# dr-tony-lin/CarND-MPC-Project

Hardware: AMD Instinct MI355X
Metric: MPC solves/sec (batch) at N=10 dt=0.1 (higher is better)
Workload: dtype f64

## Files before the change

### carnd-mpc-project_amd/csrc/mpc_core.h

```cpp
#ifndef MPC_CORE_H
#define MPC_CORE_H

#include <math.h>
#include <stdint.h>
#include <type_traits>

#include "mpc_amd.h"

#if defined(__HIPCC__)
#define MPC_HD __host__ __device__ __forceinline__
#else
#define MPC_HD inline
#endif
#if defined(__HIPCC__) || defined(__clang__)
#define MPC_UNROLL _Pragma("unroll")
#define MPC_STAGE_LOOP _Pragma("clang loop unroll(disable)")
#else
#define MPC_UNROLL _Pragma("GCC unroll 8")
#define MPC_STAGE_LOOP
#endif

namespace mpc {

template <class R> struct Layout;
// ... 13 lines not shown
    SOC_C = 0, SOC_D = 6, SOC_SZ = SOC_D + D_N
  };
  static_assert((int)GAIN_SZ <= (int)L::IT_SZ, "the gains must fit an iterate slot");
  static_assert(L::F_ZL % L::G == 0 && L::F_ZU == L::F_ZL + 4 && L::F_U == L::F_S + 6, "blocks the forward sweep fetches");
};

MPC_HD int64_t workspace_fields_per_instance(int N, bool f32, bool s0_rows = false) {
  return (int64_t)(N - 1 + (s0_rows ? 1 : 0)) * (f32 ? (int)Fields<float>::STAGE_SZ : (int)Fields<double>::STAGE_SZ);
}
MPC_HD int64_t soc_fields_per_instance(int N) { return (int64_t)(N - 1) * (int)Fields<double>::SOC_SZ; }

template <class R>
struct HostWorkspace {
  using F = Fields<R>;
  static constexpr bool kSocDefault = true;
  R *base;
  mutable R socbuf[(MPC_MAX_N - 1) * F::SOC_SZ] = {};
  MPC_HD R &soc(int k, int f) const { return socbuf[k * F::SOC_SZ + f]; }
  MPC_HD R &it(int k, int I, int f) const { return base[k * F::STAGE_SZ + I + f]; }
  MPC_HD R getD(int k, int j) const { return base[k * F::STAGE_SZ + F::F_D + j]; }
  MPC_HD void setD(int k, int j, R v) const { base[k * F::STAGE_SZ + F::F_D + j] = v; }
  template <int F0, int COUNT> MPC_HD void store_run(int k, int I, const R *v) const {
    for (int j = 0; j < COUNT; j++) base[k * F::STAGE_SZ + I + F0 + j] = v[j];
  }
  MPC_HD void stage_fetch_it(int, int, int) const {}
  MPC_HD void stage_fetch_itf(int, int, int) const {}
  MPC_HD void stage_fetch_d(int, int) const {}
  template <int N> MPC_HD void stage_wait() const {}
  MPC_HD void stage_drain() const {}
  MPC_HD R sit(int, int k, int I, int j) const { return base[k * F::STAGE_SZ + I + j]; }
  MPC_HD R sx(int, int k, int Fo, int j) const { return base[k * F::STAGE_SZ + Fo + j]; }
  MPC_HD void stage_fetch_g(int, int, int) const {}
  MPC_HD R sg(int, int k, int J, int j) const { return base[k * F::STAGE_SZ + J + F::F_GK + j]; }
};

#if defined(__HIPCC__)
#if defined(__HIP_DEVICE_COMPILE__)
typedef __attribute__((address_space(1))) double gdouble;
typedef __attribute__((address_space(1))) float gfloat;
typedef __attribute__((address_space(1))) char gchar;
typedef __attribute__((address_space(3))) double ldouble;
typedef __attribute__((address_space(3))) float lfloat;
typedef __attribute__((address_space(3))) char lchar;
#else
typedef double gdouble;
typedef float gfloat;
typedef char gchar;
typedef double ldouble;
typedef float lfloat;
typedef char lchar;
#endif
#if defined(__HIP_DEVICE_COMPILE__)
__device__ __forceinline__ unsigned mpc_uniform(unsigned x) {
  unsigned s = (unsigned)__builtin_amdgcn_readfirstlane((int)x);
  asm volatile("" : "+s"(s));
  return s;
}
#define MPC_UNIFORM(x) mpc_uniform((unsigned)(x))
#else
#define MPC_UNIFORM(x) ((unsigned)(x))
#endif
template <class R> struct AddrSpace;
template <> struct AddrSpace<double> { typedef gdouble g; typedef ldouble l; };
template <> struct AddrSpace<float> { typedef gfloat g; typedef lfloat l; };

template <bool STAGING, class R, bool LANE_ROWS = false>
struct TiledWorkspace {
  static_assert(!(STAGING && LANE_ROWS), "LDS-DMA copies record k of every lane from a scalar base: per-lane rows are not staged");
  using F = Fields<R>;
  typedef typename AddrSpace<R>::g greal;
  typedef typename AddrSpace<R>::l lreal;
  static constexpr bool kSocDefault = false;
  greal *tile;
  lreal *lbuf;
  int lane;
  static constexpr unsigned G = F::G;
  static constexpr unsigned GROUPS = F::STAGE_SZ / F::G;
  static_assert(F::STAGE_SZ % F::G == 0 && F::IT_SZ % F::G == 0, "whole groups");
  MPC_HD gchar *row(int k, int f) const {
    if constexpr (LANE_ROWS) return (gchar *)tile + (((unsigned)k * GROUPS + ((unsigned)f / G)) * 1024u + ((unsigned)f % G) * (unsigned)sizeof(R));
    else return (gchar *)tile + MPC_UNIFORM(((unsigned)k * GROUPS + ((unsigned)f / G)) * 1024u + ((unsigned)f % G) * (unsigned)sizeof(R));
  }
  MPC_HD unsigned voff(int I) const { return (unsigned)lane * 16u + ((unsigned)I / G) * 1024u; }
  MPC_HD greal &it(int k, int I, int f) const { return *(greal *)(row(k, f) + voff(I)); }
  template <int F0, int COUNT> MPC_HD void store_run(int k, int I, const R *v) const {
    static_assert(F0 % F::G == 0 && COUNT % F::G == 0, "whole groups");
    typedef R __attribute__((ext_vector_type(16 / sizeof(R)))) vec;
    typedef __attribute__((address_space(1))) vec gvec;
    MPC_UNROLL
    for (int g = 0; g < COUNT / (int)G; g++) {
      vec x;
      MPC_UNROLL
      for (int e = 0; e < (int)G; e++) x[e] = v[g * (int)G + e];
      *(gvec *)(row(k, F0 + g * (int)G) + voff(I)) = x;
    }
  }
  MPC_HD R getD(int k, int j) const { return it(k, 0, F::F_D + j); }
  MPC_HD void setD(int k, int j, R v) const { it(k, 0, F::F_D + j) = v; }
#if defined(MPC_DMA_NT) && MPC_DMA_NT
// ... 18 lines not shown
        asm volatile("s_mov_b32 m0, %2\n\tglobal_load_lds_dwordx4 %0, %1" MPC_DMA_POLICY "\n\tglobal_load_lds_dwordx4 %0, %1 offset:1024" MPC_DMA_POLICY "\n\t"
                     "global_load_lds_dwordx4 %0, %1 offset:2048" MPC_DMA_POLICY
                     :: "v"(vo), "s"(src), "s"(m0v) : "memory", "m0");
      else if (q0 + 2 == n)
        asm volatile("s_mov_b32 m0, %2\n\tglobal_load_lds_dwordx4 %0, %1" MPC_DMA_POLICY "\n\tglobal_load_lds_dwordx4 %0, %1 offset:1024" MPC_DMA_POLICY
                     :: "v"(vo), "s"(src), "s"(m0v) : "memory", "m0");
      else
        asm volatile("s_mov_b32 m0, %2\n\tglobal_load_lds_dwordx4 %0, %1" MPC_DMA_POLICY :: "v"(vo), "s"(src), "s"(m0v) : "memory", "m0");
    }
#endif
  }
  MPC_HD void stage_fetch_it(int buf, int k, int I) const { if (STAGING) dma<F::STG_IT_OPS>(buf, k, I, 0, 0); }
  MPC_HD void stage_fetch_itf(int buf, int k, int I) const {
    if (STAGING) { dma<8 / F::G>(buf, k, I, F::F_S, F::F_S / F::G); dma<8 / F::G>(buf, k, I, F::F_ZL, F::F_ZL / F::G); }
  }
  MPC_HD void stage_fetch_d(int buf, int k) const { if (STAGING) dma<F::STG_D_OPS>(buf, k, 0, F::F_D, F::STG_IT_OPS); }
  MPC_HD void stage_fetch_g(int buf, int k, int J) const { if (STAGING) dma<F::STG_X_OPS>(buf, k, J, F::F_GK, F::STG_IT_OPS); }
  MPC_HD void stage_drain() const {
#if !defined(MPC_NO_DRAIN)
    stage_wait<0>();
#endif
  }
  template <int N> MPC_HD void stage_wait() const {
#if defined(__HIP_DEVICE_COMPILE__)
    if (STAGING) asm volatile("s_waitcnt vmcnt(%0)" ::"n"(N) : "memory");
#endif
  }
  MPC_HD R sl(int buf, int j) const {
    return lbuf[(((unsigned)buf * F::STG_SLOT + ((unsigned)j / G)) * 64u + (unsigned)lane) * G + ((unsigned)j % G)];
  }
  MPC_HD R sit(int buf, int k, int I, int j) const { return STAGING ? sl(buf, j) : (R)it(k, I, j); }
  MPC_HD R sx(int buf, int k, int Fo, int j) const { return STAGING ? sl(buf, F::IT_SZ + j) : (R)it(k, 0, Fo + j); }
  MPC_HD R sg(int buf, int k, int J, int j) const { return STAGING ? sl(buf, F::IT_SZ + j) : (R)it(k, J, F::F_GK + j); }
};
template <bool STAGING, class R>
struct TiledSocWorkspace : TiledWorkspace<STAGING, R> {
  using F = Fields<R>;
  typedef typename AddrSpace<R>::g greal;
  static constexpr bool kSocDefault = true;
  greal *soc_tile;
  MPC_HD greal &soc(int k, int f) const {
    constexpr unsigned G = F::G;
    static_assert(F::SOC_SZ % F::G == 0, "whole groups");
    return soc_tile[(((unsigned)k * (F::SOC_SZ / G) + (unsigned)f / G) * 64u + (unsigned)this->lane) * G + (unsigned)f % G];
  }
};

template <class R, int LANES>
struct LdsWorkspace {
  using F = Fields<R>;
  typedef typename AddrSpace<R>::l lreal;
  static constexpr bool kSocDefault = false;
  lreal *base;
  int lane;
  MPC_HD lreal &it(int k, int I, int f) const { return base[(unsigned)((k * F::STAGE_SZ + I + f) * LANES + lane)]; }
  MPC_HD R getD(int k, int j) const { return it(k, 0, F::F_D + j); }
  MPC_HD void setD(int k, int j, R v) const { it(k, 0, F::F_D + j) = v; }
  template <int F0, int COUNT> MPC_HD void store_run(int k, int I, const R *v) const {
    MPC_UNROLL
    for (int j = 0; j < COUNT; j++) it(k, I, F0 + j) = v[j];
  }
  MPC_HD void stage_fetch_it(int, int, int) const {}
  MPC_HD void stage_fetch_itf(int, int, int) const {}
  MPC_HD void stage_fetch_d(int, int) const {}
  MPC_HD void stage_fetch_g(int, int, int) const {}
  template <int N> MPC_HD void stage_wait() const {}
  MPC_HD void stage_drain() const {}
  MPC_HD R sit(int, int k, int I, int j) const { return it(k, I, j); }
  MPC_HD R sx(int, int k, int Fo, int j) const { return it(k, 0, Fo + j); }
  MPC_HD R sg(int, int k, int J, int j) const { return it(k, J, F::F_GK + j); }
};
template <class R, int LANES>
struct LdsSocWorkspace : LdsWorkspace<R, LANES> {
  using F = Fields<R>;
  typedef typename AddrSpace<R>::l lreal;
  static constexpr bool kSocDefault = true;
  lreal *soc_base;
  MPC_HD lreal &soc(int k, int f) const { return soc_base[(unsigned)((k * F::SOC_SZ + f) * LANES + this->lane)]; }
};
#endif

MPC_HD double frcp(double x) {
#if defined(__HIP_DEVICE_COMPILE__)
  double r = __builtin_amdgcn_rcp(x);
  double e = fma(-x, r, 1.0);
  r = fma(r, e, r);
  e = fma(-x, r, 1.0);
  r = fma(r, e, r);
  return r;
#else
  return 1.0 / x;
#endif
}
#if defined(__HIP_DEVICE_COMPILE__)
template <int LPI> __device__ __forceinline__ int wave_bcast_i(int x, int lane, int base) {
  if constexpr (LPI >= 64) return __builtin_amdgcn_readlane(x, lane);
  else return __builtin_amdgcn_ds_bpermute((base + lane) << 2, x);
}
template <int LPI> __device__ __forceinline__ double wave_bcast(double x, int lane, int base) {
  const int lo = wave_bcast_i<LPI>(__double2loint(x), lane, base), hi = wave_bcast_i<LPI>(__double2hiint(x), lane, base);
  return __hiloint2double(hi, lo);
}
template <int LPI> __device__ __forceinline__ float wave_bcast(float x, int lane, int base) { return __int_as_float(wave_bcast_i<LPI>(__float_as_int(x), lane, base)); }
// ... 626 lines not shown
    R sn[6];
    MPC_UNROLL
    for (int i = 0; i < 6; i++) sn[i] = ws.sit(0, M - 1, I, F_S + i);
    {
      R Hpp, Hvv, Hee, Hcc, gp, gv, ge, gc;
      state_terms(sn[2], sn[3], sn[4], sn[5], ws.sit(0, M - 1, I, F_ZL + 0), ws.sit(0, M - 1, I, F_ZU + 0),
                  ws.sit(0, M - 1, I, F_ZL + 1), ws.sit(0, M - 1, I, F_ZU + 1), Hpp, Hvv, Hee, Hcc, gp, gv, ge, gc);
      Pm[0][0] = hxy; Pm[1][1] = hxy; Pm[2][2] = Hpp + dw; Pm[3][3] = Hvv + dw; Pm[4][4] = Hee + dw;
      Pcc = Hcc + dw; p[2] = gp; p[3] = gv; p[4] = ge; pc = gc;
    }
    R delta = ws.sit(0, M - 1, I, F_U + 0), acc = ws.sit(0, M - 1, I, F_U + 1);
    R lx = ws.sit(0, M - 1, I, F_LAM + 0), ly = ws.sit(0, M - 1, I, F_LAM + 1), lp = ws.sit(0, M - 1, I, F_LAM + 2);
    R lc = ws.sit(0, M - 1, I, F_LAM + 4), le = ws.sit(0, M - 1, I, F_LAM + 5);
    R zld = ws.sit(0, M - 1, I, F_ZL + 2), zud = ws.sit(0, M - 1, I, F_ZU + 2);
    R zla = ws.sit(0, M - 1, I, F_ZL + 3), zua = ws.sit(0, M - 1, I, F_ZU + 3);
    if (M >= 2) ws.stage_fetch_it(1, M - 2, I);
    MPC_STAGE_LOOP
    for (int k = M - 1; k >= 0; --k) {
      R sk[6];
      R zlp = 0, zup = 0, zlv = 0, zuv = 0, delprev = 0;
      const int bk = (M - k) & 1;
      if (k > 0) {
        if (k >= 2) {
          ws.stage_fetch_it(bk ^ 1, k - 2, I);
          if (k == M - 1) ws.template stage_wait<STG_IT_OPS>();
          else ws.template stage_wait<STG_IT_OPS + ST_BACKWARD>();
        } else ws.template stage_wait<0>();
        MPC_UNROLL
        for (int i = 0; i < 6; i++) sk[i] = ws.sit(bk, k - 1, I, F_S + i);
        zlp = ws.sit(bk, k - 1, I, F_ZL + 0); zup = ws.sit(bk, k - 1, I, F_ZU + 0);
        zlv = ws.sit(bk, k - 1, I, F_ZL + 1); zuv = ws.sit(bk, k - 1, I, F_ZU + 1);
        delprev = ws.sit(bk, k - 1, I, F_U + 0);
      } else {
        MPC_UNROLL
        for (int i = 0; i < 6; i++) sk[i] = st[i];
        sk[2] = p0; sk[3] = v0k;
      }
      const R v = sk[3];
      LinR L;
      linearise(sk, delta, acc, sn, L);
      soc_residual(soc, k, L);
      const R sp = L.sp, cp = L.cp, se = L.se, ce = L.ce, fp = L.fp, g1 = L.g1, h3 = L.h3, fpp = L.fpp;
      const R r0 = rsc * L.c[0], r1 = rsc * L.c[1], r2 = rsc * L.c[2], r3 = rsc * L.c[3], rc = rsc * L.c[4], r4 = rsc * L.c[5];
      const R vdt = v * dt;
      const R Axp = -vdt * sp, Axv = dt * cp, Ayp = vdt * cp, Ayv = dt * sp, Apv = delta * dtLf;
      const R Acx = fp, Acv = dt * se, Ace = vdt * ce, Aex = -g1, Bp = v * dtLf;
      R t[6];
      MPC_UNROLL
      for (int i = 0; i < 6; i++)
        t[i] = p[i] + PM(i, 0) * r0 + PM(i, 1) * r1 + PM(i, 2) * r2 + PM(i, 3) * r3 + PM(i, 4) * r4;
      const R tc = pc + Pcc * rc;
      R qt[7];
      MPC_GT(t, tc, qt);
      const R isld = frcp1(delta - dl), isud = frcp1(du - delta), isla = frcp1(acc - al), isua = frcp1(au - acc);
      R ddl = 0, Hdd = 0;
      if (k >= 1 && !lsm) { ddl = delta - delprev; Hdd = df * R(2.0) * wdd; }
      const R mub = lsm ? R(0.0) : mu;
      const R gdel = df * R(2.0) * wd * delta + Hdd * ddl + mub * (isud - isld);
      const R gacc = mub * (isua - isla);
      const R rt_d = qt[5] + gdel, rt_a = qt[6] + gacc;
      const R Sgd = lsm ? R(1.0) : df * R(2.0) * wd + zld * isld + zud * isud, Sga = lsm ? R(1.0) : zla * isla + zua * isua;
      R w5[6], w6[6];
      MPC_UNROLL
      for (int i = 0; i < 6; i++) { w5[i] = Bp * (PM(i, 2) + PM(i, 4)) + PM(i, 5); w6[i] = dt * PM(i, 3); }
      if (k == 0) {
        R o5[7], o6[7];
        MPC_GT(w5, R(0.0), o5);
        MPC_GT(w6, R(0.0), o6);
        const R Rdd = o5[5] + Sgd + dw;
        const R Rda = o6[5];
        const R Raa = o6[6] + Sga + dw;
        const R det = Rdd * Raa - Rda * Rda;
        if (!(Rdd > R(0.0)) || !(det > R(0.0))) return false;
        const R idet = frcp1(det);
        const R i11 = Raa * idet, i12 = -Rda * idet, i22 = Rdd * idet;
        const R Sd2 = o5[2], Sd3 = o5[3] - (lp + le) * dtLf, Sa2 = o6[2], Sa3 = o6[3];
        R gn[GAIN_SZ] = {};
        gn[2] = -(i11 * Sd2 + i12 * Sa2); gn[3] = -(i11 * Sd3 + i12 * Sa3);
        gn[6 + 2] = -(i12 * Sd2 + i22 * Sa2); gn[6 + 3] = -(i12 * Sd3 + i22 * Sa3);
        gn[GK_N] = -(Raa * rt_d - Rda * rt_a) * idet; gn[GK_N + 1] = -(-Rda * rt_d + Rdd * rt_a) * idet;
        ws.template store_run<F_GK, GAIN_SZ>(0, J, gn);
        break;
      }
      R Mx[7][7];
      {
        R w[6], o[7];
        MPC_UNROLL
        for (int i = 0; i < 6; i++) w[i] = PM(i, 0) + Aex * PM(i, 4);
        MPC_GT(w, Pcc * Acx, o);
        MPC_UNROLL
        for (int i = 0; i < 7; i++) Mx[i][0] = o[i];
        MPC_UNROLL
        for (int i = 0; i < 6; i++) w[i] = PM(i, 1);
        MPC_GT(w, -Pcc, o);
        MPC_UNROLL
        for (int i = 0; i < 7; i++) Mx[i][1] = o[i];
        MPC_UNROLL
        for (int i = 0; i < 6; i++) w[i] = Axp * PM(i, 0) + Ayp * PM(i, 1) + PM(i, 2) + PM(i, 4);
        MPC_GT(w, R(0.0), o);
        MPC_UNROLL
        for (int i = 0; i < 7; i++) Mx[i][2] = o[i];
        MPC_UNROLL
        for (int i = 0; i < 6; i++) w[i] = Axv * PM(i, 0) + Ayv * PM(i, 1) + Apv * (PM(i, 2) + PM(i, 4)) + PM(i, 3);
        MPC_GT(w, Pcc * Acv, o);
        MPC_UNROLL
        for (int i = 0; i < 7; i++) Mx[i][3] = o[i];
        {
          const R wcs = Pcc * Ace;
          Mx[0][4] = Acx * wcs; Mx[1][4] = -wcs; Mx[2][4] = R(0.0); Mx[3][4] = Acv * wcs; Mx[4][4] = Ace * wcs;
          Mx[5][4] = R(0.0); Mx[6][4] = R(0.0);
        }
        MPC_GT(w5, R(0.0), o);
        MPC_UNROLL
        for (int i = 0; i < 7; i++) Mx[i][5] = o[i];
// ... 134 lines not shown
    if (s0_rows && !lsm) {
      const R xs0[2] = {p0, v0k}, lo0[2] = {yl, vl}, hi0[2] = {yu, vu}, dx0[2] = {s0d2, s0d3};
      MPC_UNROLL
      for (int b = 0; b < 2; b++) {
        const R isl0 = frcp1(xs0[b] - lo0[b]), isu0 = frcp1(hi0[b] - xs0[b]);
        const R zl0 = s0_z(I, b, 0), zu0 = s0_z(I, b, 1);
        const R dzl = mu * isl0 - zl0 - zl0 * isl0 * dx0[b];
        const R dzu = mu * isu0 - zu0 + zu0 * isu0 * dx0[b];
        rzmax = mpc_max(rzmax, mpc_max(-dzl * frcp1(zl0), -dzu * frcp1(zu0)));
      }
    }
    amax = (rmax > tau) ? tau / rmax : R(1.0);
    az = (rzmax > tau) ? tau / rzmax : R(1.0);
  }

  MPC_HD void forward(bool soc = false) {
    if constexpr (WAVE) { forward_wave(soc); return; }
    const int I = it(cur), J = it(1 - cur);
    R d0 = 0, d1 = 0, d2 = 0, d3 = 0, d5 = 0;
    R ddprev = 0, delprev = 0;
    R rmax = R(0.0), rzmax = R(0.0);
    const R rsc = lsm ? R(0.0) : R(1.0);
    dphi = R(0.0); dxinf = R(0.0); xinf = R(0.0);
    R sk[6];
    load_state(0, I, sk);
    d2 = rsc * (st[2] - p0); d3 = rsc * (st[3] - v0k);
    if (d2 != R(0.0) || d3 != R(0.0)) {
      const R islp = frcp1(p0 - yl), isup = frcp1(yu - p0), islv = frcp1(v0k - vl), isuv = frcp1(vu - v0k);
      rmax = mpc_max(mpc_max(-d2 * islp, d2 * isup), mpc_max(-d3 * islv, d3 * isuv));
      dphi = mu * ((isup - islp) * d2 + (isuv - islv) * d3);
      dxinf = mpc_max(mpc_abs(d2), mpc_abs(d3));
    }
    const R s0d2 = d2, s0d3 = d3;
    ws.stage_drain();
    ws.stage_fetch_itf(0, 0, I);
    ws.stage_fetch_g(0, 0, J);
    R z0lp = R(1.0), z0up = R(1.0), z0lv = R(1.0), z0uv = R(1.0);
    if (s0_rows) { z0lp = s0_z(I, 0, 0); z0up = s0_z(I, 0, 1); z0lv = s0_z(I, 1, 0); z0uv = s0_z(I, 1, 1); }
    MPC_STAGE_LOOP
    for (int k = 0; k < M; ++k) {
      const int bf = k & 1;
      if (k + 1 < M) {
        ws.stage_fetch_itf(bf ^ 1, k + 1, I);
        ws.stage_fetch_g(bf ^ 1, k + 1, J);
        if (k == 0) ws.template stage_wait<STG_ITF_OPS + STG_X_OPS>();
        else ws.template stage_wait<STG_ITF_OPS + STG_X_OPS + ST_FORWARD>();
      } else ws.template stage_wait<0>();
      R sn[6];
      MPC_UNROLL
      for (int i = 0; i < 6; i++) sn[i] = ws.sit(bf, k, I, F_S + i);
      const R v = sk[3];
      const R delta = ws.sit(bf, k, I, F_U + 0), acc = ws.sit(bf, k, I, F_U + 1);
      LinR L;
      linearise(sk, delta, acc, sn, L);
      soc_residual(soc, k, L);
      R dd = ws.sg(bf, k, J, GK_N + 0), da = ws.sg(bf, k, J, GK_N + 1);
      dd += ws.sg(bf, k, J, 0) * d0 + ws.sg(bf, k, J, 1) * d1 + ws.sg(bf, k, J, 2) * d2 + ws.sg(bf, k, J, 3) * d3 +
            ws.sg(bf, k, J, 4) * d5 + ws.sg(bf, k, J, 5) * ddprev;
      da += ws.sg(bf, k, J, 6) * d0 + ws.sg(bf, k, J, 7) * d1 + ws.sg(bf, k, J, 8) * d2 + ws.sg(bf, k, J, 9) * d3 +
            ws.sg(bf, k, J, 10) * d5 + ws.sg(bf, k, J, 11) * ddprev;
      const R vdt = v * dt, Apv = delta * dtLf, Bp = v * dtLf;
      const R n0 = d0 - vdt * L.sp * d2 + dt * L.cp * d3 - rsc * L.c[0];
      const R n1 = d1 + vdt * L.cp * d2 + dt * L.sp * d3 - rsc * L.c[1];
      const R n2 = d2 + Apv * d3 + Bp * dd - rsc * L.c[2];
      const R n3 = d3 + dt * da - rsc * L.c[3];
      const R n4 = L.fp * d0 - d1 + dt * L.se * d3 + vdt * L.ce * d5 - rsc * L.c[4];
      const R n5 = -L.g1 * d0 + d2 + Apv * d3 + Bp * dd - rsc * L.c[5];
      {
        const R dn[D_N] = {n0, n1, n2, n3, n4, n5, dd, da};
        ws.template store_run<F_D, D_N>(k, 0, dn);
      }
      const R q2 = n2, q3 = n3, q4 = n4, q5 = n5, qd = dd, qa = da;
      const R xs[4] = {sn[2], sn[3], delta, acc};
      const R lo[4] = {yl, vl, dl, al}, hi[4] = {yu, vu, du, au};
      const R dx[4] = {q2, q3, qd, qa};
      MPC_UNROLL
      for (int b = 0; b < 4; b++) {
        const R isl = frcp1(xs[b] - lo[b]), isu = frcp1(hi[b] - xs[b]);
        const R zl = ws.sit(bf, k, I, F_ZL + b), zu = ws.sit(bf, k, I, F_ZU + b);
        rmax = mpc_max(rmax, mpc_max(-dx[b] * isl, dx[b] * isu));
        const R dzl = mu * isl - zl - zl * isl * dx[b];
        const R dzu = mu * isu - zu + zu * isu * dx[b];
        rzmax = mpc_max(rzmax, mpc_max(-dzl * frcp1(zl), -dzu * frcp1(zu)));
        dphi += mu * (isu - isl) * dx[b];
      }
      R g = R(2.0) * wc * sn[4] * q4 + R(2.0) * we * sn[5] * q5 + R(2.0) * wv * (sn[3] - vref) * q3 + R(2.0) * wd * delta * qd;
      if (k > 0) g += R(2.0) * wdd * (delta - delprev) * (qd - ddprev);
      dphi += df * g;
      dxinf = mpc_max(dxinf, mpc_max(mpc_max(mpc_max(mpc_abs(n0), mpc_abs(n1)), mpc_max(mpc_abs(n2), mpc_abs(n3))),
                               mpc_max(mpc_max(mpc_abs(n4), mpc_abs(n5)), mpc_max(mpc_abs(dd), mpc_abs(da)))));
      xinf = mpc_max(xinf, mpc_max(mpc_max(mpc_abs(sn[0]), mpc_abs(sn[1])), mpc_max(mpc_abs(sn[3]), mpc_abs(sn[4]))));
      d0 = n0; d1 = n1; d2 = n2; d3 = n3; d5 = n5; ddprev = dd; delprev = delta;
      MPC_UNROLL
      for (int i = 0; i < 6; i++) sk[i] = sn[i];
    }
    if (s0_rows && !lsm) {
      const R xs0[2] = {p0, v0k}, lo0[2] = {yl, vl}, hi0[2] = {yu, vu}, dx0[2] = {s0d2, s0d3};
      const R zl0[2] = {z0lp, z0lv}, zu0[2] = {z0up, z0uv};
      MPC_UNROLL
      for (int b = 0; b < 2; b++) {
        const R isl = frcp1(xs0[b] - lo0[b]), isu = frcp1(hi0[b] - xs0[b]);
        const R dzl = mu * isl - zl0[b] - zl0[b] * isl * dx0[b];
        const R dzu = mu * isu - zu0[b] + zu0[b] * isu * dx0[b];
        rzmax = mpc_max(rzmax, mpc_max(-dzl * frcp1(zl0[b]), -dzu * frcp1(zu0[b])));
      }
    }
    amax = (rmax > tau) ? tau / rmax : R(1.0);
    az = (rzmax > tau) ? tau / rzmax : R(1.0);
  }

  MPC_HD EvalR costate_trial(R dw, R alpha, R alpha_l, R alpha_z, bool with_costate, R &lmax) {
    const int I = it(cur), J = it(1 - cur);
    const R hxy = (lsm ? R(1.0) : R(0.0)) + dw;
    EvalR Ev;
    Ev.theta = 0; Ev.cinf = 0; Ev.f = 0; Ev.L = 0; Ev.dinf = 0; Ev.cmin = IC::huge; Ev.cmax = 0; Ev.lsum = 0; Ev.zsum = 0; Ev.du0 = 0; Ev.ok = true;
    lmax = R(0.0);
    const R ksm = IC::kappa_sigma * mu, ksi = mu * (R(1.0) / IC::kappa_sigma);
    R sn_o[6] = {0, 0, 0, 0, 0, 0}, del_o = 0, acc_o = 0, lx = 0, ly = 0, lp = 0, lc = 0, le = 0, ddk = 0;
    R L0 = 0, L1 = 0, L2 = 0, L3 = 0, L4 = 0, L5 = 0;
    R sn_t[6] = {0, 0, 0, 0, 0, 0}, ln_t[6] = {0, 0, 0, 0, 0, 0}, del_t = 0, acc_t = 0, del_nx = 0;
    R zdl_t = 0, zdu_t = 0, zal_t = 0, zau_t = 0;
    ws.stage_drain();
    ws.stage_fetch_it(0, M - 1, I);
    ws.stage_fetch_d(0, M - 1);
    R c_l0 = 0, c_l1 = 0, c_l2 = 0, c_l3 = 0, c_l4 = 0, c_l5 = 0, c_zlp = 0, c_zup = 0, c_zlv = 0, c_zuv = 0;
    if (s0_rows) {
      c_l0 = s0_lam(I, 0); c_l1 = s0_lam(I, 1); c_l2 = s0_lam(I, 2); c_l3 = s0_lam(I, 3); c_l4 = s0_lam(I, 4); c_l5 = s0_lam(I, 5);
      c_zlp = s0_z(I, 0, 0); c_zup = s0_z(I, 0, 1); c_zlv = s0_z(I, 1, 0); c_zuv = s0_z(I, 1, 1);
    }
    auto step_k = [&](auto kz_, const int k) {
      constexpr bool KZ = decltype(kz_)::value;
        const int bk = (M - k) & 1;
        R s_o[6], s_t[6], lam_t[6] = {0, 0, 0, 0, 0, 0};
        R zs0 = 0, zs1 = 0, zs2 = 0, zs3 = 0;
        R n_del_o = 0, n_acc_o = 0, n_ddk = 0, lo0 = 0, lo1 = 0, lo2 = 0, lo4 = 0, lo5 = 0;
        R n_del_t = 0, n_acc_t = 0, n_zdl = 0, n_zdu = 0, n_zal = 0, n_zau = 0;
        if constexpr (!KZ) {
          if (k >= 2) {
            ws.stage_fetch_it(bk ^ 1, k - 2, I);
            ws.stage_fetch_d(bk ^ 1, k - 2);
            if (k == M) ws.template stage_wait<STG_IT_OPS + STG_D_OPS>();
            else ws.template stage_wait<STG_IT_OPS + STG_D_OPS + ST_TRIAL>();
          } else ws.template stage_wait<0>();
          const int r = k - 1;
          R ds[6];
          MPC_UNROLL
          for (int i = 0; i < 6; i++) { s_o[i] = ws.sit(bk, r, I, F_S + i); ds[i] = ws.sx(bk, r, F_D, D_S + i); }
          const R lo3 = ws.sit(bk, r, I, F_LAM + 3);
          lo0 = ws.sit(bk, r, I, F_LAM + 0); lo1 = ws.sit(bk, r, I, F_LAM + 1); lo2 = ws.sit(bk, r, I, F_LAM + 2);
          lo4 = ws.sit(bk, r, I, F_LAM + 4); lo5 = ws.sit(bk, r, I, F_LAM + 5);
          n_del_o = ws.sit(bk, r, I, F_U + 0); n_acc_o = ws.sit(bk, r, I, F_U + 1);
          const R ddel = ws.sx(bk, r, F_D, D_U + 0), dacc = ws.sx(bk, r, F_D, D_U + 1);
          n_ddk = ddel;
          if (r == 0) Ev.du0 = mpc_max(mpc_abs(ddel), mpc_abs(dacc));
          R dl0 = 0, dl1 = 0, dl2 = 0, dl3 = 0, dl4 = 0, dl5 = 0;
          if (with_costate) {
            R Hpp, Hvv, Hee, Hcc, gp, gv, ge, gc;
            state_terms(s_o[2], s_o[3], s_o[4], s_o[5], ws.sit(bk, r, I, F_ZL + 0), ws.sit(bk, r, I, F_ZU + 0),
                        ws.sit(bk, r, I, F_ZL + 1), ws.sit(bk, r, I, F_ZU + 1), Hpp, Hvv, Hee, Hcc, gp, gv, ge, gc);
            R n0, n1, n2, n3, n4, n5;
            if (k == M) {
              n0 = -(hxy * ds[0]);
              n1 = -(hxy * ds[1]);
              n2 = -(gp + (Hpp + dw) * ds[2]);
              n3 = -(gv + (Hvv + dw) * ds[3]);
              n4 = -(gc + (Hcc + dw) * ds[4]);
              n5 = -(ge + (Hee + dw) * ds[5]);
            } else {
              const R v = s_o[3];
              LinR L;
              linearise(s_o, del_o, acc_o, sn_o, L);
              const R sp = L.sp, cp = L.cp, se = L.se, ce = L.ce, fp = L.fp, g1 = L.g1, h3 = L.h3, fpp = L.fpp;
              const R vdt = v * dt, Apv = del_o * dtLf;
// ... 666 lines not shown
      ws.it(M, Ic, F_ZL + 0) = a(43); ws.it(M, Ic, F_ZU + 0) = a(44); ws.it(M, Ic, F_ZL + 1) = a(45); ws.it(M, Ic, F_ZU + 1) = a(46);
    }
    iters = iter; phase = PH_DIR;
  }

  MPC_HD void promoted() {
    phase = PH_EVAL0; keep_theta = true; ls_start = false; nf = 0; n_polish = 0; acc_count = 0; out_step = out_prev = IC::huge;
    alpha = alpha_l = alpha_z = dw_cur = R(0.0);
    p0 = st[2]; v0k = st[3];
  }

  MPC_HD void begin(bool ls) {
    cur = 0; mu = IC::mu_init; tau = mpc_max(IC::tau_min, R(1.0) - mu); nf = 0; iters = 0; n_reg = 0; lsm = false;
    phase = ls ? PH_LS : PH_EVAL0; iter = 0; ls_start = ls; tiny = false; n_polish = 0; acc_count = 0; no_restart = false; out_step = out_prev = IC::huge;
    p0 = pushed(st[2], yl, yu); v0k = pushed(st[3], vl, vu);
    if (s0_rows) s0_reset(IT0);
    alpha = alpha_l = alpha_z = dw_cur = R(0.0);
    theta_max = theta_min = dw_last = R(0.0);
    theta_k = phi_k = pth = pdp = amin = R(0.0);
  }

  MPC_HD int line_search_failed() {
    if ((kCanPromote && promote_mu > R(0.0))) { promote_clean = false; return MPC_PROMOTE; }
    const R E0 = kkt_error(E, R(0.0));
    if (sizeof(R) == 4 && E0 <= R(10.0) * tol) return MPC_STATUS_SUCCESS;
    if (n_polish > 0 && converged_at(E, E0)) return MPC_STATUS_SUCCESS;
    if (acceptable_at(E, E0)) return MPC_STATUS_ACCEPTABLE;
    if (sizeof(R) == 8 && P.acceptable_iter > 0 && E.cinf <= R(1e-2) * tol) no_restart = true;
    return MPC_STATUS_LINESEARCH;
  }

  MPC_HD int step() {
    const R mu_floor = sizeof(R) == 8 ? tol / R(10.0) : tol / R(25.0);
    if (phase == PH_LS || phase == PH_DIR || phase == PH_REG || (kSoc && phase == PH_SOC)) {
      if (phase != PH_REG) { dw_try = R(0.0); reg_tries = 0; }
      if (phase == PH_DIR) {
        iters = iter;
        const R E0 = kkt_error(E, R(0.0));
        if (!(E0 == E0)) return MPC_STATUS_NUMERIC;
        if ((kCanPromote && promote_mu > R(0.0)) && (E0 <= tol || iter >= promote_cap)) { promote_clean = E0 <= tol; return MPC_PROMOTE; }
        if (converged_at(E, E0)) {
          if (!P.polish || n_polish >= kMaxPolish || iter >= P.max_iter || (mu <= mu_floor && out_step <= out_tol))
            return MPC_STATUS_SUCCESS;
          ++n_polish;
          if (mu > mu_floor) { mu = mu_floor; tau = mpc_max(IC::tau_min, R(1.0) - mu); nf = 0; }
        } else if (acceptable_at(E, E0)) {
          if (++acc_count >= P.acceptable_iter) return MPC_STATUS_ACCEPTABLE;
        } else acc_count = 0;
        if (iter >= P.max_iter) return MPC_STATUS_MAXITER;
        while (kkt_error(E, mu) <= IC::kappa_eps * mu && mu > mu_floor) {
          mu = mpc_max(mu_floor, mpc_min(IC::kappa_mu * mu, mu * mpc_sqrt(mu)));
          if (P.polish && mu < R(3.0) * mu_floor) mu = mu_floor;
          tau = mpc_max(IC::tau_min, R(1.0) - mu);
          nf = 0;
        }
        if ((kCanPromote && promote_mu > R(0.0)) && mu <= promote_mu) { promote_clean = true; return MPC_PROMOTE; }
#if defined(MPC_TRACE) && !defined(__HIP_DEVICE_COMPILE__)
        printf("it %3d f=%.8g theta=%.3e dinf=%.3e cmin=%.2e cmax=%.2e mu=%.2e E0=%.3e nf=%d\n", iter, E.f, E.theta,
               E.dinf, E.cmin, E.cmax, mu, E0, nf);
#endif
      }
      bool soc = false;
      if constexpr (kSoc) {
        soc = phase == PH_SOC;
        if (soc) soc_prepare();
      }
      lsm = (phase == PH_LS);
      R dw = dw_try;
      if constexpr (kSoc) { if (soc) dw = dw_cur; }
      bool okb = true;
      if (!backward(dw, soc)) {
        if (lsm) okb = false;
        else if (soc) return soc_give_up();
        else {
          if (dw == R(0.0)) dw = (dw_last == R(0.0)) ? IC::dw_0 : mpc_max(IC::dw_min, IC::kw_minus * dw_last);
          else dw *= (dw_last == R(0.0)) ? IC::kw_plus_bar : IC::kw_plus;
          if (dw > IC::dw_max || ++reg_tries > 100) { promote_clean = false; return (kCanPromote && promote_mu > R(0.0)) ? (int)MPC_PROMOTE : (int)MPC_STATUS_LINESEARCH; }
          dw_try = dw; phase = PH_REG;
          return MPC_RUNNING;
        }
      }
      if (phase == PH_REG) phase = PH_DIR;
      if (okb) forward(soc);
      dw_cur = dw;
      if (soc) {
        if constexpr (kSoc) { this->soc_as = amax; dphi = this->soc_dphi; dxinf = this->soc_dxinf; }
        alpha = amax; alpha_l = amax; alpha_z = az;
      } else if (phase == PH_LS) {
        if (!okb) { lsm = false; ls_start = false; phase = PH_EVAL0; return MPC_RUNNING; }
        alpha = R(0.0); alpha_l = R(1.0); alpha_z = R(0.0);
      } else {
        if (dw > R(0.0)) { dw_last = dw; n_reg++; }
        theta_k = E.theta; phi_k = df * E.f - mu * E.L;
        pth = hpow(theta_k, IC::s_theta);
        pdp = (dphi < R(0.0)) ? hpow(-dphi, IC::s_phi) : R(0.0);
        if (dphi < R(0.0)) {
          const R t3 = (theta_k <= theta_min) ? IC::delta_sw * pth / pdp : IC::gamma_theta;
          amin = IC::gamma_alpha * mpc_min(mpc_min(IC::gamma_theta, IC::gamma_phi * theta_k / (-dphi)), t3);
        } else amin = IC::gamma_alpha * IC::gamma_theta;
        tiny = dxinf <= R(10.0) * IC::eps * mpc_max(R(1.0), xinf);
        alpha = amax; alpha_l = amax; alpha_z = az;
      }
    }
    R lmax;
    const EvalR T = costate_trial(dw_cur, alpha, alpha_l, alpha_z, phase != PH_EVAL0, lmax);
    if (phase == PH_EVAL0) {
      E = T; cur = 1 - cur;

      if (!E.ok) return MPC_STATUS_NUMERIC;
      if (!keep_theta) { theta_max = R(1e4) * mpc_max(R(1.0), E.theta); theta_min = R(1e-4) * mpc_max(R(1.0), E.theta); }
      keep_theta = false;
      phase = ls_start ? PH_LS : PH_DIR;
      return MPC_RUNNING;
    }
    if (phase == PH_LS) {
      lsm = false; ls_start = false;
      if (lmax <= R(1000.0)) {
        E = T; cur = 1 - cur;

        if (!E.ok) return MPC_STATUS_NUMERIC;
        theta_max = R(1e4) * mpc_max(R(1.0), E.theta); theta_min = R(1e-4) * mpc_max(R(1.0), E.theta);
        phase = PH_DIR;
      } else phase = PH_EVAL0;
      return MPC_RUNNING;
    }
    bool accepted = false, ftype = false;
    R a_test = alpha;
    if constexpr (kSoc) { if (phase == PH_SOC) a_test = this->soc_a0; }
    if (tiny) { accepted = T.ok; ftype = true; }
    else if (T.ok) {
      const R phi_t = df * T.f - mu * T.L;
      const R eps_phi = R(10.0) * IC::eps * mpc_abs(phi_k);
      if (T.theta < theta_max && !filter_rejects(T.theta, phi_t)) {
        const bool sw = dphi < R(0.0) && a_test * pdp > IC::delta_sw * pth;
        const bool armijo = phi_t - phi_k - eps_phi <= IC::eta_phi * a_test * dphi;
        if (theta_k <= theta_min && sw) {
          if (armijo) accepted = true;
        } else if (T.theta <= (R(1.0) - IC::gamma_theta) * theta_k ||
// ... 330 lines not shown
```

### carnd-mpc-project_amd/csrc/mpc_solver.hip

```cpp
#include <hip/hip_runtime.h>

#include <cstdio>
#include <cstdlib>
#include <cstring>
#include <chrono>
#include <mutex>
#include <string>
#include <thread>
#include <tuple>
#include <vector>

#include "mpc_core.h"
#include "mpc_run_core.h"
#include "mpc_drive_core.h"
#include "mpc_take_key.h"

namespace {

thread_local std::string g_last_error;

#define MPC_HIP_CHECK(expr)                                                              \
  do {                                                                                   \
    hipError_t e_ = (expr);                                                              \
    if (e_ != hipSuccess) {                                                              \
// ... 226 lines not shown
template <bool MODEL, class Phase>
__device__ __forceinline__ decltype(auto) drive_model_vals(const MpcParams &P, const Phase &T, int64_t i) {
  if constexpr (MODEL) return mpc::model_vals_of(P, T.model, T.ld_model, i);
  else return (P);
}

template <class SV>
__device__ __forceinline__ int64_t park_for_next_phase(const MpcPhase &T, const SV &S, int64_t i, int attempt, int it_total, bool from_scratch) {
  const int64_t pos = (int64_t)atomicAdd(T.n_out, 1);
  T.out_inst[pos] = (int32_t)i;
  T.out_src[pos] = (int32_t)(blockIdx.x * 64u + threadIdx.x);
  double *pk = T.out_park + pos;
  const int64_t lp = T.ld_park;
  S.park([pk, lp](int q) -> double & { return pk[q * lp]; }, attempt, it_total);
  pk[35 * lp] = from_scratch ? 1.0 : 0.0;
  return pos;
}

template <bool STAGING, class R, class RIO = R, class RSRC = RIO, bool SOC = false, bool WARM = false, bool ROLL = false, bool MODEL = false,
          bool HORIZON = false, bool DRIVE = false>
__global__ __launch_bounds__(kBlock, 1) void mpc_solve_kernel(
    const MpcParams P, const int64_t B, const int64_t ld, const int64_t ldo, const RIO *__restrict__ state,
    const RIO *__restrict__ coeffs, const RIO *__restrict__ yaw_lo, const RIO *__restrict__ yaw_hi,
    const RIO *__restrict__ weights, RIO *__restrict__ out, RIO *__restrict__ traj,
    int32_t *__restrict__ status, int32_t *__restrict__ iters, R *__restrict__ wsbase,
    const int64_t tile_reals,
    const MpcPhaseOf<ROLL, WARM, MODEL, HORIZON, DRIVE> T) {
  extern __shared__ double smem[];
  static_assert(!DRIVE || (ROLL && !HORIZON && !SOC), "track driving: a ROLL build without HORIZON and SOC");
  static_assert(!HORIZON || (MODEL && !STAGING && !SOC), "per-instance horizon: a MODEL build without staging and SOC");
  static_assert(!WARM || (sizeof(R) == 8 && std::is_same<R, RIO>::value && std::is_same<R, RSRC>::value && !SOC), "warm start: the plain fp64 solve only");
  static_assert(!ROLL || (sizeof(R) == 8 && std::is_same<R, RIO>::value && std::is_same<R, RSRC>::value && !SOC), "fused rollout: the plain fp64 solve only");
  static_assert(!MODEL || (sizeof(R) == 8 && std::is_same<R, RIO>::value && std::is_same<R, RSRC>::value), "per-instance model values: the fp64 solve only");
  using WS = std::conditional_t<SOC, mpc::TiledSocWorkspace<STAGING, R>, mpc::TiledWorkspace<STAGING, R, HORIZON>>;
  using SV = mpc::Solver<WS, R, 0, SOC>;
  using FL = mpc::Fields<R>;
  static_assert(SV::PARK_N == kParkRows, "park buffer rows");
  WS ws;
  ws.tile = (typename WS::greal *)(wsbase + (int64_t)blockIdx.x * tile_reals);
  if constexpr (SOC) ws.soc_tile = (typename WS::greal *)((R *)T.soc_ws + (int64_t)blockIdx.x * (P.N - 1) * FL::SOC_SZ * 64);
  ws.lane = threadIdx.x;
  ws.lbuf = (typename WS::lreal *)smem;
  if (T.zero_next && blockIdx.x == 0 && threadIdx.x < kCounterInts) T.zero_next[threadIdx.x] = 0;
  SV S(P, ws);
  if (T.promote_out) S.promote_mu = (R)P.mixed_switch_mu;
  int64_t i = 0;
  bool have = false, more = true, fin = false;
  bool queue_full = false;
  bool col_busy = false;
  int attempt = 0, it_total = 0, passes = 0, fin_status = 0, waited = 0, cooldown = 0;
  int step = 0;
  int drive_k = 0, drive_k_prev = 0;
  (void)drive_k; (void)drive_k_prev;
  const int64_t n_work = T.resume ? (int64_t)*T.n_in : B;
  (void)col_busy; (void)cooldown; (void)step;
  for (;;) {
#if defined(__HIP_DEVICE_COMPILE__)
    bool want_compact = false;
    int cnt[8] = {0, 0, 0, 0, 0, 0, 0, 0}, g_min = 0;
    if ((STAGING || HORIZON) && T.compact_gap > 0) {
      if (MPC_WAVE_ANY(more) && (int64_t)__hip_atomic_load(T.take, __ATOMIC_RELAXED, __HIP_MEMORY_SCOPE_AGENT) >= n_work) more = false;
      if (!MPC_WAVE_ANY(more)) {
        if (cooldown > 0) --cooldown;
        else {
          const unsigned long long live = __builtin_amdgcn_ballot_w64(have);
          const int nl = __builtin_popcountll(live);
          int g_now = 0;
// ... 2586 lines not shown
```

Baseline: 50.07 million.

## Carry staged LDS buffers across backward, forward and costate sweeps

```diff
diff --git a/carnd-mpc-project_amd/csrc/mpc_core.h b/carnd-mpc-project_amd/csrc/mpc_core.h
--- a/carnd-mpc-project_amd/csrc/mpc_core.h
+++ b/carnd-mpc-project_amd/csrc/mpc_core.h
@@ -69,6 +69,11 @@
   MPC_HD R sx(int, int k, int Fo, int j) const { return base[k * F::STAGE_SZ + Fo + j]; }
   MPC_HD void stage_fetch_g(int, int, int) const {}
   MPC_HD R sg(int, int k, int J, int j) const { return base[k * F::STAGE_SZ + J + F::F_GK + j]; }
+  static constexpr bool kCarry = false;
+  MPC_HD void stage_fetch_lam(int, int, int) const {}
+  MPC_HD void stage_put_g(int, const R *) const {}
+  MPC_HD void stage_put_d(int, const R *) const {}
+  MPC_HD bool stage_all(bool) const { return false; }
 };
 
 #if defined(__HIPCC__)
@@ -101,7 +106,7 @@
 template <> struct AddrSpace<double> { typedef gdouble g; typedef ldouble l; };
 template <> struct AddrSpace<float> { typedef gfloat g; typedef lfloat l; };
 
-template <bool STAGING, class R, bool LANE_ROWS = false>
+template <bool STAGING, class R, bool LANE_ROWS = false, bool CARRY = true>
 struct TiledWorkspace {
   static_assert(!(STAGING && LANE_ROWS), "LDS-DMA copies record k of every lane from a scalar base: per-lane rows are not staged");
   using F = Fields<R>;
@@ -186,6 +191,24 @@
   MPC_HD R sit(int buf, int k, int I, int j) const { return STAGING ? sl(buf, j) : (R)it(k, I, j); }
   MPC_HD R sx(int buf, int k, int Fo, int j) const { return STAGING ? sl(buf, F::IT_SZ + j) : (R)it(k, 0, Fo + j); }
   MPC_HD R sg(int buf, int k, int J, int j) const { return STAGING ? sl(buf, F::IT_SZ + j) : (R)it(k, J, F::F_GK + j); }
+  static constexpr bool kCarry = STAGING && CARRY;
+  MPC_HD void stage_fetch_lam(int buf, int k, int I) const {
+    if (STAGING) dma<(F::F_ZL - F::F_LAM) / F::G>(buf, k, I, F::F_LAM, F::F_LAM / F::G);
+  }
+  template <int COUNT> MPC_HD void stage_put_n(int buf, const R *v) const {
+    MPC_UNROLL
+    for (int j = 0; j < COUNT; j++)
+      lbuf[(((unsigned)buf * F::STG_SLOT + ((unsigned)(F::IT_SZ + j) / G)) * 64u + (unsigned)lane) * G + ((unsigned)(F::IT_SZ + j) % G)] = v[j];
+  }
+  MPC_HD void stage_put_g(int buf, const R *v) const { if (kCarry) stage_put_n<F::GAIN_SZ>(buf, v); }
+  MPC_HD void stage_put_d(int buf, const R *v) const { if (kCarry) stage_put_n<F::D_N>(buf, v); }
+  MPC_HD bool stage_all(bool p) const {
+#if defined(__HIP_DEVICE_COMPILE__)
+    return kCarry && __builtin_amdgcn_ballot_w64(!p) == 0ull;
+#else
+    return false;
+#endif
+  }
 };
 template <bool STAGING, class R>
 struct TiledSocWorkspace : TiledWorkspace<STAGING, R> {
@@ -223,6 +246,11 @@
   MPC_HD R sit(int, int k, int I, int j) const { return it(k, I, j); }
   MPC_HD R sx(int, int k, int Fo, int j) const { return it(k, 0, Fo + j); }
   MPC_HD R sg(int, int k, int J, int j) const { return it(k, J, F::F_GK + j); }
+  static constexpr bool kCarry = false;
+  MPC_HD void stage_fetch_lam(int, int, int) const {}
+  MPC_HD void stage_put_g(int, const R *) const {}
+  MPC_HD void stage_put_d(int, const R *) const {}
+  MPC_HD bool stage_all(bool) const { return false; }
 };
 template <class R, int LANES>
 struct LdsSocWorkspace : LdsWorkspace<R, LANES> {
@@ -915,6 +943,9 @@
         zlv = ws.sit(bk, k - 1, I, F_ZL + 1); zuv = ws.sit(bk, k - 1, I, F_ZU + 1);
         delprev = ws.sit(bk, k - 1, I, F_U + 0);
       } else {
+        if constexpr (WS::kCarry) {
+          if (M >= 2) { ws.stage_fetch_itf(M & 1, 1, I); ws.stage_fetch_g(M & 1, 1, J); }
+        }
         MPC_UNROLL
         for (int i = 0; i < 6; i++) sk[i] = st[i];
         sk[2] = p0; sk[3] = v0k;
@@ -963,6 +994,7 @@
         gn[6 + 2] = -(i12 * Sd2 + i22 * Sa2); gn[6 + 3] = -(i12 * Sd3 + i22 * Sa3);
         gn[GK_N] = -(Raa * rt_d - Rda * rt_a) * idet; gn[GK_N + 1] = -(-Rda * rt_d + Rdd * rt_a) * idet;
         ws.template store_run<F_GK, GAIN_SZ>(0, J, gn);
+        ws.stage_put_g((M - 1) & 1, gn);
         break;
       }
       R Mx[7][7];
@@ -1163,15 +1195,18 @@
       dxinf = mpc_max(mpc_abs(d2), mpc_abs(d3));
     }
     const R s0d2 = d2, s0d3 = d3;
-    ws.stage_drain();
-    ws.stage_fetch_itf(0, 0, I);
-    ws.stage_fetch_g(0, 0, J);
+    if constexpr (!WS::kCarry) {
+      ws.stage_drain();
+      ws.stage_fetch_itf(0, 0, I);
+      ws.stage_fetch_g(0, 0, J);
+    }
     R z0lp = R(1.0), z0up = R(1.0), z0lv = R(1.0), z0uv = R(1.0);
     if (s0_rows) { z0lp = s0_z(I, 0, 0); z0up = s0_z(I, 0, 1); z0lv = s0_z(I, 1, 0); z0uv = s0_z(I, 1, 1); }
     MPC_STAGE_LOOP
     for (int k = 0; k < M; ++k) {
-      const int bf = k & 1;
-      if (k + 1 < M) {
+      const int bf = WS::kCarry ? (M - 1 - k) & 1 : k & 1;
+      if (WS::kCarry && k == 0) {
+      } else if (k + 1 < M) {
         ws.stage_fetch_itf(bf ^ 1, k + 1, I);
         ws.stage_fetch_g(bf ^ 1, k + 1, J);
         if (k == 0) ws.template stage_wait<STG_ITF_OPS + STG_X_OPS>();
@@ -1200,6 +1235,13 @@
       {
         const R dn[D_N] = {n0, n1, n2, n3, n4, n5, dd, da};
         ws.template store_run<F_D, D_N>(k, 0, dn);
+        if constexpr (WS::kCarry) {
+          if (k == M - 1) {
+            ws.stage_put_d(bf, dn);
+            ws.stage_fetch_lam(bf, k, I);
+            if (M >= 2) { ws.stage_fetch_it(bf ^ 1, M - 2, I); ws.stage_fetch_d(bf ^ 1, M - 2); }
+          }
+        }
       }
       const R q2 = n2, q3 = n3, q4 = n4, q5 = n5, qd = dd, qa = da;
       const R xs[4] = {sn[2], sn[3], delta, acc};
@@ -1240,7 +1282,7 @@
     az = (rzmax > tau) ? tau / rzmax : R(1.0);
   }
 
-  MPC_HD EvalR costate_trial(R dw, R alpha, R alpha_l, R alpha_z, bool with_costate, R &lmax) {
+  MPC_HD EvalR costate_trial(R dw, R alpha, R alpha_l, R alpha_z, bool with_costate, R &lmax, bool from_forward = false) {
     const int I = it(cur), J = it(1 - cur);
     const R hxy = (lsm ? R(1.0) : R(0.0)) + dw;
     EvalR Ev;
@@ -1251,9 +1293,12 @@
     R L0 = 0, L1 = 0, L2 = 0, L3 = 0, L4 = 0, L5 = 0;
     R sn_t[6] = {0, 0, 0, 0, 0, 0}, ln_t[6] = {0, 0, 0, 0, 0, 0}, del_t = 0, acc_t = 0, del_nx = 0;
     R zdl_t = 0, zdu_t = 0, zal_t = 0, zau_t = 0;
-    ws.stage_drain();
-    ws.stage_fetch_it(0, M - 1, I);
-    ws.stage_fetch_d(0, M - 1);
+    const bool carry = WS::kCarry && ws.stage_all(from_forward);
+    if (!carry) {
+      ws.stage_drain();
+      ws.stage_fetch_it(0, M - 1, I);
+      ws.stage_fetch_d(0, M - 1);
+    }
     R c_l0 = 0, c_l1 = 0, c_l2 = 0, c_l3 = 0, c_l4 = 0, c_l5 = 0, c_zlp = 0, c_zup = 0, c_zlv = 0, c_zuv = 0;
     if (s0_rows) {
       c_l0 = s0_lam(I, 0); c_l1 = s0_lam(I, 1); c_l2 = s0_lam(I, 2); c_l3 = s0_lam(I, 3); c_l4 = s0_lam(I, 4); c_l5 = s0_lam(I, 5);
@@ -1268,8 +1313,10 @@
         R n_del_t = 0, n_acc_t = 0, n_zdl = 0, n_zdu = 0, n_zal = 0, n_zau = 0;
         if constexpr (!KZ) {
           if (k >= 2) {
-            ws.stage_fetch_it(bk ^ 1, k - 2, I);
-            ws.stage_fetch_d(bk ^ 1, k - 2);
+            if (!(carry && k == M)) {
+              ws.stage_fetch_it(bk ^ 1, k - 2, I);
+              ws.stage_fetch_d(bk ^ 1, k - 2);
+            }
             if (k == M) ws.template stage_wait<STG_IT_OPS + STG_D_OPS>();
             else ws.template stage_wait<STG_IT_OPS + STG_D_OPS + ST_TRIAL>();
           } else ws.template stage_wait<0>();
@@ -2002,6 +2049,7 @@
 
   MPC_HD int step() {
     const R mu_floor = sizeof(R) == 8 ? tol / R(10.0) : tol / R(25.0);
+    bool from_forward = false;
     if (phase == PH_LS || phase == PH_DIR || phase == PH_REG || (kSoc && phase == PH_SOC)) {
       if (phase != PH_REG) { dw_try = R(0.0); reg_tries = 0; }
       if (phase == PH_DIR) {
@@ -2051,7 +2099,7 @@
         }
       }
       if (phase == PH_REG) phase = PH_DIR;
-      if (okb) forward(soc);
+      if (okb) { forward(soc); from_forward = true; }
       dw_cur = dw;
       if (soc) {
         if constexpr (kSoc) { this->soc_as = amax; dphi = this->soc_dphi; dxinf = this->soc_dxinf; }
@@ -2073,7 +2121,7 @@
       }
     }
     R lmax;
-    const EvalR T = costate_trial(dw_cur, alpha, alpha_l, alpha_z, phase != PH_EVAL0, lmax);
+    const EvalR T = costate_trial(dw_cur, alpha, alpha_l, alpha_z, phase != PH_EVAL0, lmax, from_forward);
     if (phase == PH_EVAL0) {
       E = T; cur = 1 - cur;
 
diff --git a/carnd-mpc-project_amd/csrc/mpc_solver.hip b/carnd-mpc-project_amd/csrc/mpc_solver.hip
--- a/carnd-mpc-project_amd/csrc/mpc_solver.hip
+++ b/carnd-mpc-project_amd/csrc/mpc_solver.hip
@@ -282,7 +282,7 @@
   static_assert(!WARM || (sizeof(R) == 8 && std::is_same<R, RIO>::value && std::is_same<R, RSRC>::value && !SOC), "warm start: the plain fp64 solve only");
   static_assert(!ROLL || (sizeof(R) == 8 && std::is_same<R, RIO>::value && std::is_same<R, RSRC>::value && !SOC), "fused rollout: the plain fp64 solve only");
   static_assert(!MODEL || (sizeof(R) == 8 && std::is_same<R, RIO>::value && std::is_same<R, RSRC>::value), "per-instance model values: the fp64 solve only");
-  using WS = std::conditional_t<SOC, mpc::TiledSocWorkspace<STAGING, R>, mpc::TiledWorkspace<STAGING, R, HORIZON>>;
+  using WS = std::conditional_t<SOC, mpc::TiledSocWorkspace<STAGING, R>, mpc::TiledWorkspace<STAGING, R, HORIZON, !DRIVE>>;
   using SV = mpc::Solver<WS, R, 0, SOC>;
   using FL = mpc::Fields<R>;
   static_assert(SV::PARK_N == kParkRows, "park buffer rows");
```

Result: slower. 46.36 million (-7.4%).
